# santimont/brpc-github-actions

Measured on AMD Instinct MI355X. Metric: echo QPS + p99 latency (rpc_press, 32B & 64KB body) at 1/2/4/8 MI355X, higher is better.
Workload: dtype uint8

## Files before the change

### brpc_amd/csrc/pb/descriptor.cc

```cpp
#include "pb/descriptor.h"

#include <string>

#include "pb/message.h"

namespace mrpc {
namespace pb {

Descriptor::~Descriptor() {
    if (owns_prototype) delete prototype;
}

const char* FieldTypeName(FieldType t) {
    switch (t) {
    case FieldType::DOUBLE: return "double";
    case FieldType::FLOAT: return "float";
    case FieldType::INT64: return "int64";
    case FieldType::UINT64: return "uint64";
    case FieldType::INT32: return "int32";
    case FieldType::FIXED64: return "fixed64";
    case FieldType::FIXED32: return "fixed32";
    case FieldType::BOOL: return "bool";
    case FieldType::STRING: return "string";
    case FieldType::GROUP: return "group";
// ... 28 lines not shown
size_t CppTypeAlign(CppType t) {
    switch (t) {
    case CppType::BOOL: return 1;
    case CppType::INT32:
    case CppType::UINT32:
    case CppType::ENUM:
    case CppType::FLOAT: return 4;
    default: return 8;
    }
}

std::string ToJsonName(const std::string& s) {
    std::string out;
    bool up = false;
    for (char c : s) {
        if (c == '_') {
            up = true;
        } else if (up) {
            out.push_back((char)toupper((unsigned char)c));
            up = false;
        } else {
            out.push_back(c);
        }
    }
    return out;
}

bool FieldDescriptor::is_map() const { return is_repeated() && message_type && message_type->map_entry; }

const EnumValueDescriptor* EnumDescriptor::FindValueByNumber(int n) const {
    for (auto& v : values) {
        if (v.number == n) return &v;
    }
    return nullptr;
}

const EnumValueDescriptor* EnumDescriptor::FindValueByName(const std::string& s) const {
    for (auto& v : values) {
        if (v.name == s) return &v;
    }
    return nullptr;
}

void Descriptor::BuildIndex() {
    _by_number.clear();
    _by_number_sparse.clear();
    _by_name.clear();
    for (size_t i = 0; i < fields.size(); ++i) {
        FieldDescriptor& f = fields[i];
        f.index = (int)i;
        f.containing_type = this;
        if (f.json_name.empty()) f.json_name = ToJsonName(f.name);
        if (f.number > 0 && f.number < 256) {
            if ((int)_by_number.size() <= f.number) _by_number.resize(f.number + 1, 0);
            _by_number[f.number] = (int)i + 1;
        } else {
            _by_number_sparse[f.number] = (int)i;
        }
        _by_name[f.name] = (int)i;
    }
}

const FieldDescriptor* Descriptor::FindFieldByNumber(int n) const {
    if (n > 0 && n < (int)_by_number.size()) {
        int i = _by_number[n];
        return i ? &fields[i - 1] : nullptr;
    }
    auto it = _by_number_sparse.find(n);
    return it == _by_number_sparse.end() ? nullptr : &fields[it->second];
}

const FieldDescriptor* Descriptor::FindFieldByName(const std::string& s) const {
    auto it = _by_name.find(s);
    return it == _by_name.end() ? nullptr : &fields[it->second];
}

const FieldDescriptor* Descriptor::FindFieldByJsonName(const std::string& s) const {
    for (auto& f : fields) {
        if (f.json_name == s) return &f;
    }
    return nullptr;
}

Message* Descriptor::NewMessage() const {
    if (factory) return factory();
    if (prototype) return prototype->New();
    return nullptr;
}

const MethodDescriptor* ServiceDescriptor::FindMethodByName(const std::string& n) const {
    for (auto& m : methods) {
        if (m.name == n) return &m;
    }
    return nullptr;
}

DescriptorPool* DescriptorPool::generated_pool() {
    static DescriptorPool* p = new DescriptorPool;
    return p;
}

void DescriptorPool::add_message(Descriptor* d) {
    _messages[d->full_name] = d;
    for (Descriptor* n : d->nested_types) add_message(n);
    for (EnumDescriptor* e : d->enum_types) _enums[e->full_name] = e;
}

void DescriptorPool::AddFile(FileDescriptor* f) {
    std::lock_guard<std::mutex> g(_mu);
    _files.emplace_back(f);
    _file_by_name[f->name] = f;
    for (Descriptor* d : f->message_types) add_message(d);
    for (EnumDescriptor* e : f->enum_types) _enums[e->full_name] = e;
    for (ServiceDescriptor* s : f->services) _services[s->full_name] = s;
}

const FileDescriptor* DescriptorPool::FindFileByName(const std::string& n) const {
    std::lock_guard<std::mutex> g(_mu);
    auto it = _file_by_name.find(n);
    return it == _file_by_name.end() ? nullptr : it->second;
}

static std::string strip_dot(const std::string& s) { return (!s.empty() && s[0] == '.') ? s.substr(1) : s; }

const Descriptor* DescriptorPool::FindMessageTypeByName(const std::string& n) const {
    std::lock_guard<std::mutex> g(_mu);
    auto it = _messages.find(strip_dot(n));
    return it == _messages.end() ? nullptr : it->second;
}

const EnumDescriptor* DescriptorPool::FindEnumTypeByName(const std::string& n) const {
    std::lock_guard<std::mutex> g(_mu);
    auto it = _enums.find(strip_dot(n));
    return it == _enums.end() ? nullptr : it->second;
}

const ServiceDescriptor* DescriptorPool::FindServiceByName(const std::string& n) const {
    std::lock_guard<std::mutex> g(_mu);
    auto it = _services.find(strip_dot(n));
    return it == _services.end() ? nullptr : it->second;
}

const MethodDescriptor* DescriptorPool::FindMethodByName(const std::string& n) const {
    std::string s = strip_dot(n);
    size_t dot = s.rfind('.');
    if (dot == std::string::npos) return nullptr;
    const ServiceDescriptor* sd = FindServiceByName(s.substr(0, dot));
    return sd ? sd->FindMethodByName(s.substr(dot + 1)) : nullptr;
}

std::vector<const FileDescriptor*> DescriptorPool::files() const {
    std::lock_guard<std::mutex> g(_mu);
    std::vector<const FileDescriptor*> out;
    for (auto& f : _files) out.push_back(f.get());
    return out;
}

std::vector<const ServiceDescriptor*> DescriptorPool::services() const {
    std::lock_guard<std::mutex> g(_mu);
    std::vector<const ServiceDescriptor*> out;
    for (auto& kv : _services) out.push_back(kv.second);
    return out;
}

}
}
// ... 1 lines not shown
```

### brpc_amd/csrc/pb/descriptor.h

```cpp
#pragma once

#include <atomic>

#include <cstdint>
#include <map>
#include <memory>
#include <mutex>
#include <string>
#include <vector>

namespace mrpc {
namespace pb {

class Message;
class Descriptor;
class EnumDescriptor;
class FileDescriptor;
class ServiceDescriptor;

enum class FieldType : uint8_t {
    DOUBLE = 1, FLOAT = 2, INT64 = 3, UINT64 = 4, INT32 = 5, FIXED64 = 6, FIXED32 = 7, BOOL = 8,
    STRING = 9, GROUP = 10, MESSAGE = 11, BYTES = 12, UINT32 = 13, ENUM = 14, SFIXED32 = 15,
    SFIXED64 = 16, SINT32 = 17, SINT64 = 18,
};
// ... 12 lines not shown
    return i < 19 ? kMap[i] : CppType::INT32;
}
size_t CppTypeSize(CppType t);
size_t CppTypeAlign(CppType t);

struct EnumValueDescriptor {
    std::string name;
    int number;
};

class EnumDescriptor {
public:
    std::string name;
    std::string full_name;
    const FileDescriptor* file = nullptr;
    std::vector<EnumValueDescriptor> values;
    const EnumValueDescriptor* FindValueByNumber(int n) const;
    const EnumValueDescriptor* FindValueByName(const std::string& s) const;
};

class FieldDescriptor {
public:
    std::string name;
    std::string json_name;
    int number = 0;
    FieldType type = FieldType::INT32;
    Label label = Label::OPTIONAL;
    bool packed = false;
    bool proto3_implicit = false;
    std::string type_name;
    const Descriptor* message_type = nullptr;
    const EnumDescriptor* enum_type = nullptr;
    const Descriptor* containing_type = nullptr;
    int index = 0;
    int oneof_index = -1;
    bool has_default = false;
    std::string default_str;
    int64_t default_int = 0;
    uint64_t default_uint = 0;
    double default_double = 0;
    std::string default_string;
    uint32_t offset = 0;
    int32_t has_bit = -1;
    std::map<std::string, std::string> options;

    bool is_repeated() const { return label == Label::REPEATED; }
    bool is_required() const { return label == Label::REQUIRED; }
    bool is_map() const;
    CppType cpp_type() const { return CppTypeOf(type); }
    bool is_packable() const { return cpp_type() != CppType::STRING && cpp_type() != CppType::MESSAGE; }
};

class Descriptor {
public:
    std::string name;
    std::string full_name;
    const FileDescriptor* file = nullptr;
    const Descriptor* containing_type = nullptr;
    std::vector<FieldDescriptor> fields;
    std::vector<std::string> oneof_names;
    std::vector<Descriptor*> nested_types;
    std::vector<EnumDescriptor*> enum_types;
    bool map_entry = false;
    bool proto3 = false;
    uint32_t has_bits_offset = 0;
    uint32_t num_has_bits = 0;
    uint32_t object_size = 0;
    Message* (*factory)() = nullptr;
    const Message* prototype = nullptr;
    bool owns_prototype = false;
    std::atomic<const void*> mcpack_handler{nullptr};
    Descriptor() = default;
    Descriptor(const Descriptor&) = delete;
    Descriptor& operator=(const Descriptor&) = delete;
    ~Descriptor();

    int field_count() const { return (int)fields.size(); }
    const FieldDescriptor* field(int i) const { return &fields[i]; }
    const FieldDescriptor* FindFieldByNumber(int n) const;
    const FieldDescriptor* FindFieldByName(const std::string& s) const;
    const FieldDescriptor* FindFieldByJsonName(const std::string& s) const;
    void BuildIndex();
    Message* NewMessage() const;

private:
    std::vector<int> _by_number;
    std::map<int, int> _by_number_sparse;
    std::map<std::string, int> _by_name;
};

class MethodDescriptor {
public:
    std::string name;
    std::string full_name;
    const ServiceDescriptor* service = nullptr;
    const Descriptor* input_type = nullptr;
    const Descriptor* output_type = nullptr;
    std::string input_type_name;
    std::string output_type_name;
    int index = 0;
    bool client_streaming = false;
    bool server_streaming = false;
    std::map<std::string, std::string> options;
};

class ServiceDescriptor {
public:
    std::string name;
    std::string full_name;
    const FileDescriptor* file = nullptr;
    std::vector<MethodDescriptor> methods;
    std::map<std::string, std::string> options;
    int method_count() const { return (int)methods.size(); }
    const MethodDescriptor* method(int i) const { return &methods[i]; }
    const MethodDescriptor* FindMethodByName(const std::string& n) const;
};

class FileDescriptor {
public:
    std::string name;
    std::string package;
    std::string syntax = "proto2";
    std::vector<std::string> dependencies;
    std::vector<Descriptor*> message_types;
    std::vector<EnumDescriptor*> enum_types;
    std::vector<ServiceDescriptor*> services;
    std::map<std::string, std::string> options;
    std::string source;
    std::vector<std::unique_ptr<Descriptor>> owned_messages;
    std::vector<std::unique_ptr<EnumDescriptor>> owned_enums;
    std::vector<std::unique_ptr<ServiceDescriptor>> owned_services;
};

class DescriptorPool {
public:
    static DescriptorPool* generated_pool();
    void AddFile(FileDescriptor* f);
    const FileDescriptor* FindFileByName(const std::string& n) const;
    const Descriptor* FindMessageTypeByName(const std::string& full_name) const;
    const EnumDescriptor* FindEnumTypeByName(const std::string& full_name) const;
    const ServiceDescriptor* FindServiceByName(const std::string& full_name) const;
    const MethodDescriptor* FindMethodByName(const std::string& full_name) const;
    std::vector<const FileDescriptor*> files() const;
    std::vector<const ServiceDescriptor*> services() const;

private:
    void add_message(Descriptor* d);
    mutable std::mutex _mu;
    std::vector<std::unique_ptr<FileDescriptor>> _files;
    std::map<std::string, const FileDescriptor*> _file_by_name;
    std::map<std::string, const Descriptor*> _messages;
    std::map<std::string, const EnumDescriptor*> _enums;
    std::map<std::string, const ServiceDescriptor*> _services;
};

std::string ToJsonName(const std::string& field_name);

}
}
```

### brpc_amd/csrc/pb/message.cc

```cpp
#include "pb/message.h"

#include <algorithm>
#include <cmath>
#include <cstdio>
#include <sstream>

#include "base/buf.h"
#include "base/logging.h"

namespace mrpc {
namespace pb {

namespace {

template <typename T>
inline T& ref(Message* m, const FieldDescriptor* f) {
    return *reinterpret_cast<T*>(reinterpret_cast<char*>(m) + f->offset);
}
template <typename T>
inline const T& cref(const Message& m, const FieldDescriptor* f) {
    return *reinterpret_cast<const T*>(reinterpret_cast<const char*>(&m) + f->offset);
}
inline uint32_t* has_bits(Message* m) {
    return reinterpret_cast<uint32_t*>(reinterpret_cast<char*>(m) + m->GetDescriptor()->has_bits_offset);
}
inline const uint32_t* has_bits(const Message& m) {
    return reinterpret_cast<const uint32_t*>(reinterpret_cast<const char*>(&m) + m.GetDescriptor()->has_bits_offset);
}

WireType wire_type_of(FieldType t) {
    switch (t) {
    case FieldType::DOUBLE:
    case FieldType::FIXED64:
    case FieldType::SFIXED64: return WIRETYPE_FIXED64;
    case FieldType::FLOAT:
    case FieldType::FIXED32:
    case FieldType::SFIXED32: return WIRETYPE_FIXED32;
    case FieldType::STRING:
    case FieldType::BYTES:
    case FieldType::MESSAGE: return WIRETYPE_LENGTH_DELIMITED;
    case FieldType::GROUP: return WIRETYPE_START_GROUP;
    default: return WIRETYPE_VARINT;
    }
}

size_t scalar_size(FieldType t, const void* p) {
    switch (t) {
    case FieldType::DOUBLE:
    case FieldType::FIXED64:
    case FieldType::SFIXED64: return 8;
    case FieldType::FLOAT:
    case FieldType::FIXED32:
    case FieldType::SFIXED32: return 4;
    case FieldType::BOOL: return 1;
    case FieldType::INT32:
    case FieldType::ENUM: return int32_size(*(const int32_t*)p);
    case FieldType::SINT32: return varint_size(zigzag32(*(const int32_t*)p));
    case FieldType::UINT32: return varint_size(*(const uint32_t*)p);
    case FieldType::INT64: return varint_size((uint64_t)*(const int64_t*)p);
    case FieldType::SINT64: return varint_size(zigzag64(*(const int64_t*)p));
    case FieldType::UINT64: return varint_size(*(const uint64_t*)p);
    default: return 0;
    }
}

uint8_t* write_scalar(uint8_t* o, FieldType t, const void* p) {
    switch (t) {
    case FieldType::DOUBLE:
    case FieldType::FIXED64:
    case FieldType::SFIXED64: return write_fixed64(o, *(const uint64_t*)p);
    case FieldType::FLOAT:
    case FieldType::FIXED32:
    case FieldType::SFIXED32: return write_fixed32(o, *(const uint32_t*)p);
    case FieldType::BOOL: *o++ = (*(const uint8_t*)p) ? 1 : 0; return o;
    case FieldType::INT32:
    case FieldType::ENUM: return write_varint(o, (uint64_t)(int64_t)*(const int32_t*)p);
    case FieldType::SINT32: return write_varint(o, zigzag32(*(const int32_t*)p));
    case FieldType::UINT32: return write_varint(o, *(const uint32_t*)p);
    case FieldType::INT64: return write_varint(o, (uint64_t)*(const int64_t*)p);
    case FieldType::SINT64: return write_varint(o, zigzag64(*(const int64_t*)p));
    case FieldType::UINT64: return write_varint(o, *(const uint64_t*)p);
    default: return o;
    }
}

inline size_t vsize64(uint64_t v) { return (size_t)(((63 - __builtin_clzll(v | 1)) * 9 + 73) >> 6); }
size_t repeated_payload_bytes(FieldType t, const char* data, size_t n) {
    size_t s = 0;
    switch (t) {
    case FieldType::DOUBLE:
    case FieldType::FIXED64:
    case FieldType::SFIXED64: return 8 * n;
    case FieldType::FLOAT:
    case FieldType::FIXED32:
    case FieldType::SFIXED32: return 4 * n;
    case FieldType::BOOL: return n;
    case FieldType::INT32:
    case FieldType::ENUM: {
        const int32_t* v = reinterpret_cast<const int32_t*>(data);
        for (size_t i = 0; i < n; ++i) s += vsize64((uint64_t)(int64_t)v[i]);
        return s;
    }
    case FieldType::SINT32: {
        const int32_t* v = reinterpret_cast<const int32_t*>(data);
        for (size_t i = 0; i < n; ++i) s += vsize64(zigzag32(v[i]));
        return s;
    }
    case FieldType::UINT32: {
        const uint32_t* v = reinterpret_cast<const uint32_t*>(data);
        for (size_t i = 0; i < n; ++i) s += vsize64(v[i]);
        return s;
    }
    case FieldType::INT64:
    case FieldType::UINT64: {
        const uint64_t* v = reinterpret_cast<const uint64_t*>(data);
        for (size_t i = 0; i < n; ++i) s += vsize64(v[i]);
        return s;
    }
    case FieldType::SINT64: {
        const int64_t* v = reinterpret_cast<const int64_t*>(data);
        for (size_t i = 0; i < n; ++i) s += vsize64(zigzag64(v[i]));
        return s;
    }
    default: return 0;
    }
}

size_t elem_bytes(FieldType t) {
    switch (CppTypeOf(t)) {
    case CppType::BOOL: return 1;
    case CppType::INT32:
    case CppType::UINT32:
    case CppType::ENUM:
    case CppType::FLOAT: return 4;
    default: return 8;
    }
}

struct RawVec {
    const char* data;
    size_t n;
};
RawVec raw_repeated(const Message& m, const FieldDescriptor* f) {
    const char* base = reinterpret_cast<const char*>(&m) + f->offset;
    switch (f->cpp_type()) {
    case CppType::BOOL: {
        auto& v = *(const std::vector<uint8_t>*)base;
        return RawVec{(const char*)v.data(), v.size()};
    }
    case CppType::INT32:
    case CppType::ENUM: {
        auto& v = *(const std::vector<int32_t>*)base;
        return RawVec{(const char*)v.data(), v.size()};
    }
    case CppType::UINT32: {
        auto& v = *(const std::vector<uint32_t>*)base;
        return RawVec{(const char*)v.data(), v.size()};
    }
    case CppType::FLOAT: {
        auto& v = *(const std::vector<float>*)base;
        return RawVec{(const char*)v.data(), v.size()};
    }
    case CppType::INT64: {
        auto& v = *(const std::vector<int64_t>*)base;
        return RawVec{(const char*)v.data(), v.size()};
    }
    case CppType::UINT64: {
        auto& v = *(const std::vector<uint64_t>*)base;
        return RawVec{(const char*)v.data(), v.size()};
    }
    case CppType::DOUBLE: {
        auto& v = *(const std::vector<double>*)base;
        return RawVec{(const char*)v.data(), v.size()};
    }
    default: return RawVec{nullptr, 0};
    }
}

bool is_default_scalar(const Message& m, const FieldDescriptor* f) {
    switch (f->cpp_type()) {
    case CppType::BOOL: return !cref<bool>(m, f);
    case CppType::INT32:
    case CppType::ENUM: return cref<int32_t>(m, f) == 0;
    case CppType::UINT32: return cref<uint32_t>(m, f) == 0;
    case CppType::FLOAT: {
        float v = cref<float>(m, f);
        uint32_t bits;
        memcpy(&bits, &v, 4);
        return bits == 0;
    }
    case CppType::INT64: return cref<int64_t>(m, f) == 0;
    case CppType::UINT64: return cref<uint64_t>(m, f) == 0;
    case CppType::DOUBLE: {
        double v = cref<double>(m, f);
        uint64_t bits;
        memcpy(&bits, &v, 8);
        return bits == 0;
    }
    case CppType::STRING: return cref<std::string>(m, f).empty();
    case CppType::MESSAGE: return cref<Message*>(m, f) == nullptr;
    }
    return true;
}

bool field_present(const Message& m, const FieldDescriptor* f) {
    if (f->cpp_type() == CppType::MESSAGE) return cref<Message*>(m, f) != nullptr;
    if (f->has_bit >= 0) return (has_bits(m)[f->has_bit >> 5] >> (f->has_bit & 31)) & 1;
    return !is_default_scalar(m, f);
}

// ... 41 lines not shown
    ref<std::vector<T>>(m, f).push_back(v);
}

void store_number(Message* m, const FieldDescriptor* f, uint64_t raw) {
    const bool rep = f->is_repeated();
    switch (f->type) {
    case FieldType::INT32:
    case FieldType::ENUM:
    case FieldType::SFIXED32: {
        int32_t v = (int32_t)raw;
        if (rep) push_raw<int32_t>(m, f, v); else ref<int32_t>(m, f) = v;
        break;
    }
    case FieldType::SINT32: {
        int32_t v = unzigzag32((uint32_t)raw);
        if (rep) push_raw<int32_t>(m, f, v); else ref<int32_t>(m, f) = v;
        break;
    }
    case FieldType::UINT32:
    case FieldType::FIXED32: {
        uint32_t v = (uint32_t)raw;
        if (rep) push_raw<uint32_t>(m, f, v); else ref<uint32_t>(m, f) = v;
        break;
    }
    case FieldType::INT64:
    case FieldType::SFIXED64: {
        int64_t v = (int64_t)raw;
        if (rep) push_raw<int64_t>(m, f, v); else ref<int64_t>(m, f) = v;
        break;
    }
    case FieldType::SINT64: {
        int64_t v = unzigzag64(raw);
        if (rep) push_raw<int64_t>(m, f, v); else ref<int64_t>(m, f) = v;
        break;
    }
    case FieldType::UINT64:
    case FieldType::FIXED64: {
        if (rep) push_raw<uint64_t>(m, f, raw); else ref<uint64_t>(m, f) = raw;
        break;
    }
    case FieldType::BOOL: {
        uint8_t v = raw != 0;
        if (rep) push_raw<uint8_t>(m, f, v); else ref<bool>(m, f) = v;
        break;
    }
    case FieldType::FLOAT: {
        uint32_t b = (uint32_t)raw;
        float v;
        memcpy(&v, &b, 4);
        if (rep) push_raw<float>(m, f, v); else ref<float>(m, f) = v;
        break;
    }
    case FieldType::DOUBLE: {
        double v;
        memcpy(&v, &raw, 8);
        if (rep) push_raw<double>(m, f, v); else ref<double>(m, f) = v;
        break;
    }
    default: break;
    }
    if (!rep) {
        if (f->oneof_index >= 0) ClearOneofSiblings(m, f);
        set_has(m, f);
    }
}

bool read_number(CodedInput* in, FieldType t, uint64_t* out) {
    switch (wire_type_of(t)) {
    case WIRETYPE_VARINT: return in->read_varint(out);
    case WIRETYPE_FIXED32: {
        uint32_t v;
        if (!in->read_fixed32(&v)) return false;
        *out = v;
        return true;
    }
    case WIRETYPE_FIXED64: return in->read_fixed64(out);
    default: return false;
    }
}

bool parse_message(Message* m, CodedInput* in);

template <typename T, typename Conv>
bool bulk_varints(Message* m, const FieldDescriptor* f, const uint8_t* p, size_t len, Conv conv) {
    size_t n = 0;
    for (size_t i = 0; i < len; ++i) n += (p[i] >> 7) ^ 1;
    auto& vec = ref<std::vector<T>>(m, f);
    const size_t base = vec.size();
    vec.resize(base + n);
    T* out = vec.data() + base;
    CodedInput in(p, len);
    for (size_t k = 0; k < n; ++k) {
        uint64_t v;
        if (!in.read_varint(&v)) {
            vec.resize(base + k);
            return false;
        }
        out[k] = conv(v);
    }
    return in.at_limit();
}

template <typename T>
bool bulk_fixed(Message* m, const FieldDescriptor* f, const uint8_t* p, size_t len) {
    if (len % sizeof(T)) return false;
    auto& vec = ref<std::vector<T>>(m, f);
    const size_t base = vec.size();
    vec.resize(base + len / sizeof(T));
    memcpy(vec.data() + base, p, len);
    return true;
}

bool parse_packed(Message* m, const FieldDescriptor* f, const uint8_t* p, size_t len) {
    switch (f->type) {
    case FieldType::INT32:
    case FieldType::ENUM: return bulk_varints<int32_t>(m, f, p, len, [](uint64_t v) { return (int32_t)v; });
    case FieldType::SINT32:
        return bulk_varints<int32_t>(m, f, p, len, [](uint64_t v) { return unzigzag32((uint32_t)v); });
    case FieldType::UINT32: return bulk_varints<uint32_t>(m, f, p, len, [](uint64_t v) { return (uint32_t)v; });
    case FieldType::INT64: return bulk_varints<int64_t>(m, f, p, len, [](uint64_t v) { return (int64_t)v; });
    case FieldType::SINT64: return bulk_varints<int64_t>(m, f, p, len, [](uint64_t v) { return unzigzag64(v); });
    case FieldType::UINT64: return bulk_varints<uint64_t>(m, f, p, len, [](uint64_t v) { return v; });
    case FieldType::BOOL: return bulk_varints<uint8_t>(m, f, p, len, [](uint64_t v) { return (uint8_t)(v != 0); });
    case FieldType::FIXED32:
    case FieldType::SFIXED32: return f->cpp_type() == CppType::UINT32 ? bulk_fixed<uint32_t>(m, f, p, len)
                                                                      : bulk_fixed<int32_t>(m, f, p, len);
    case FieldType::FIXED64: return bulk_fixed<uint64_t>(m, f, p, len);
    case FieldType::SFIXED64: return bulk_fixed<int64_t>(m, f, p, len);
    case FieldType::FLOAT: return bulk_fixed<float>(m, f, p, len);
    case FieldType::DOUBLE: return bulk_fixed<double>(m, f, p, len);
    default: return false;
    }
}

bool parse_field(Message* m, const FieldDescriptor* f, uint32_t tag, CodedInput* in) {
    const WireType wt = (WireType)(tag & 7);
    const WireType expected = wire_type_of(f->type);
    if (f->is_repeated() && f->is_packable() && wt == WIRETYPE_LENGTH_DELIMITED) {
        uint64_t len;
        const uint8_t* p;
        if (!in->read_varint(&len) || !in->read_bytes((size_t)len, &p)) return false;
        return parse_packed(m, f, p, (size_t)len);
    }
    if (wt != expected) {
        return in->skip_field(tag, m->mutable_unknown_fields());
    }
    switch (f->cpp_type()) {
    case CppType::STRING: {
        uint64_t len;
        const uint8_t* d;
        if (!in->read_varint(&len) || !in->read_bytes((size_t)len, &d)) return false;
        if (f->is_repeated()) {
            ref<std::vector<std::string>>(m, f).emplace_back((const char*)d, (size_t)len);
        } else {
            if (f->oneof_index >= 0) ClearOneofSiblings(m, f);
            ref<std::string>(m, f).assign((const char*)d, (size_t)len);
            set_has(m, f);
        }
        return true;
    }
    case CppType::MESSAGE: {
        if (f->type == FieldType::GROUP) return in->skip_field(tag, m->mutable_unknown_fields());
        uint64_t len;
        const uint8_t* old;
        if (!in->read_varint(&len) || !in->push_limit((size_t)len, &old)) return false;
        Message* sub = f->is_repeated() ? Reflection::AddMessage(m, f) : Reflection::MutableMessage(m, f);
        if (!in->inc_depth()) return false;
        if (!parse_message(sub, in)) return false;
        in->dec_depth();
        if (!in->at_limit()) return false;
        in->pop_limit(old);
        return true;
    }
    default: {
        uint64_t v;
        if (!read_number(in, f->type, &v)) return false;
        store_number(m, f, v);
        return true;
    }
    }
}

bool parse_message(Message* m, CodedInput* in) { return m->MergePartialFromCodedInput(in); }

}


Message::~Message() {}

void Message::Clear() {
    const Descriptor* d = GetDescriptor();
    for (const FieldDescriptor& fd : d->fields) {
        const FieldDescriptor* f = &fd;
        if (f->is_repeated()) {
            clear_repeated(this, f);
        } else if (f->cpp_type() == CppType::MESSAGE) {
            Message*& sub = ref<Message*>(this, f);
            if (sub) sub->Clear();
            delete sub;
            sub = nullptr;
        } else {
            set_scalar_default(this, f);
        }
    }
    uint32_t* hb = has_bits(this);
    for (uint32_t i = 0; i < (d->num_has_bits + 31) / 32; ++i) hb[i] = 0;
    _unknown.clear();
}

size_t Message::ByteSizeLong() const {
    const Descriptor* d = GetDescriptor();
    size_t total = 0;
    for (const FieldDescriptor& fd : d->fields) {
        const FieldDescriptor* f = &fd;
        const size_t tag_size = varint_size(make_tag(f->number, WIRETYPE_VARINT));
        if (f->is_repeated()) {
            switch (f->cpp_type()) {
            case CppType::STRING: {
                const auto& v = cref<std::vector<std::string>>(*this, f);
                for (const auto& s : v) total += tag_size + varint_size(s.size()) + s.size();
                break;
            }
            case CppType::MESSAGE: {
                const auto& v = cref<RepeatedPtrBase>(*this, f);
                for (int i = 0; i < v.size(); ++i) {
                    size_t s = v.Get(i)->ByteSizeLong();
                    total += tag_size + varint_size(s) + s;
                }
                break;
            }
            default: {
                RawVec rv = raw_repeated(*this, f);
                if (rv.n == 0) break;
                const size_t data = repeated_payload_bytes(f->type, rv.data, rv.n);
                if (f->packed) total += tag_size + varint_size(data) + data;
                else total += tag_size * rv.n + data;
            }
            }
            continue;
        }
        if (!field_present(*this, f)) continue;
        switch (f->cpp_type()) {
        case CppType::STRING: {
            const auto& s = cref<std::string>(*this, f);
            total += tag_size + varint_size(s.size()) + s.size();
            break;
        }
        case CppType::MESSAGE: {
            size_t s = cref<Message*>(*this, f)->ByteSizeLong();
            total += tag_size + varint_size(s) + s;
            break;
        }
        default:
            total += tag_size + scalar_size(f->type, reinterpret_cast<const char*>(this) + f->offset);
        }
    }
    total += _unknown.size();
    _cached_size = (int)total;
    return total;
}

const void* Reflection::RepeatedScalarData(const Message& m, const FieldDescriptor* f, size_t* n, size_t* eb) {
    *n = 0;
    *eb = 0;
    if (!f->is_repeated() || f->cpp_type() == CppType::STRING || f->cpp_type() == CppType::MESSAGE) return nullptr;
    RawVec rv = raw_repeated(m, f);
    *n = rv.n;
    *eb = elem_bytes(f->type);
    return rv.data;
}

static thread_local PackedRunSink* tls_run_sink = nullptr;

PackedRunSink* SetThreadPackedRunSink(PackedRunSink* sink) {
    PackedRunSink* prev = tls_run_sink;
    tls_run_sink = sink;
    return prev;
}

bool IsVarintFieldType(FieldType t) {
    switch (t) {
    case FieldType::INT32:
    case FieldType::ENUM:
    case FieldType::SINT32:
    case FieldType::UINT32:
    case FieldType::INT64:
    case FieldType::SINT64:
    case FieldType::UINT64:
    case FieldType::BOOL: return true;
    default: return false;
    }
}

void EncodePackedRunOnHost(const PackedRun& run) {
    uint8_t* o = run.dst;
    const char* v = static_cast<const char*>(run.values);
    for (size_t i = 0; i < run.n; ++i) o = write_scalar(o, run.type, v + i * run.elem_bytes);
}

uint8_t* Message::SerializeWithCachedSizesToArray(uint8_t* o) const {
    const Descriptor* d = GetDescriptor();
    for (const FieldDescriptor& fd : d->fields) {
        const FieldDescriptor* f = &fd;
        if (f->is_repeated()) {
            switch (f->cpp_type()) {
            case CppType::STRING: {
                for (const auto& s : cref<std::vector<std::string>>(*this, f)) {
                    o = write_tag(o, f->number, WIRETYPE_LENGTH_DELIMITED);
                    o = write_varint(o, s.size());
                    memcpy(o, s.data(), s.size());
                    o += s.size();
                }
                break;
            }
            case CppType::MESSAGE: {
                const auto& v = cref<RepeatedPtrBase>(*this, f);
                for (int i = 0; i < v.size(); ++i) {
                    const Message* sub = v.Get(i);
                    o = write_tag(o, f->number, WIRETYPE_LENGTH_DELIMITED);
                    o = write_varint(o, (uint64_t)sub->GetCachedSize());
                    o = sub->SerializeWithCachedSizesToArray(o);
                }
                break;
            }
            default: {
                RawVec rv = raw_repeated(*this, f);
                if (rv.n == 0) break;
                const size_t eb = elem_bytes(f->type);
                PackedRunSink* sink = tls_run_sink;
                if (f->packed && sink && rv.n >= sink->min_elems() && IsVarintFieldType(f->type)) {
                    PackedRun run;
                    run.values = rv.data;
                    run.n = rv.n;
                    run.elem_bytes = eb;
                    run.type = f->type;
                    run.chunk_bytes.reserve((rv.n + kPackedRunChunkElems - 1) / kPackedRunChunkElems);
                    size_t data = 0;
                    for (size_t c = 0; c < rv.n; c += kPackedRunChunkElems) {
                        const size_t e = std::min(rv.n, c + kPackedRunChunkElems);
                        const size_t cb = repeated_payload_bytes(f->type, rv.data + c * eb, e - c);
                        run.chunk_bytes.push_back((uint32_t)cb);
                        data += cb;
                    }
                    o = write_tag(o, f->number, WIRETYPE_LENGTH_DELIMITED);
                    o = write_varint(o, data);
                    run.dst = o;
                    run.bytes = data;
                    o += data;
                    sink->Take(std::move(run));
                } else if (f->packed) {
                    const size_t data = repeated_payload_bytes(f->type, rv.data, rv.n);
                    o = write_tag(o, f->number, WIRETYPE_LENGTH_DELIMITED);
                    o = write_varint(o, data);
                    for (size_t i = 0; i < rv.n; ++i) o = write_scalar(o, f->type, rv.data + i * eb);
                } else {
                    const WireType wt = wire_type_of(f->type);
                    for (size_t i = 0; i < rv.n; ++i) {
                        o = write_tag(o, f->number, wt);
                        o = write_scalar(o, f->type, rv.data + i * eb);
                    }
                }
            }
            }
            continue;
        }
        if (!field_present(*this, f)) continue;
        switch (f->cpp_type()) {
        case CppType::STRING: {
            const auto& s = cref<std::string>(*this, f);
            o = write_tag(o, f->number, WIRETYPE_LENGTH_DELIMITED);
            o = write_varint(o, s.size());
            memcpy(o, s.data(), s.size());
            o += s.size();
            break;
        }
        case CppType::MESSAGE: {
            const Message* sub = cref<Message*>(*this, f);
            o = write_tag(o, f->number, WIRETYPE_LENGTH_DELIMITED);
            o = write_varint(o, (uint64_t)sub->GetCachedSize());
            o = sub->SerializeWithCachedSizesToArray(o);
            break;
        }
        default:
            o = write_tag(o, f->number, wire_type_of(f->type));
            o = write_scalar(o, f->type, reinterpret_cast<const char*>(this) + f->offset);
        }
    }
    if (!_unknown.empty()) {
        memcpy(o, _unknown.data(), _unknown.size());
        o += _unknown.size();
    }
    return o;
}

bool Message::MergePartialFromCodedInput(CodedInput* in) {
    const Descriptor* d = GetDescriptor();
    for (;;) {
        const uint32_t tag = in->read_tag();
        if (tag == 0) return true;
        if (tag == 0xFFFFFFFFu || (tag >> 3) == 0) return false;
        if ((tag & 7) == WIRETYPE_END_GROUP) return false;
        const FieldDescriptor* f = d->FindFieldByNumber((int)(tag >> 3));
        if (!f) {
            if (!in->skip_field(tag, &_unknown)) return false;
            continue;
        }
        if (!parse_field(this, f, tag, in)) return false;
    }
}

static bool is_initialized_impl(const Message& m, std::string* missing, const std::string& prefix) {
    bool ok = true;
    const Descriptor* d = m.GetDescriptor();
    for (const FieldDescriptor& fd : d->fields) {
        const FieldDescriptor* f = &fd;
        if (f->is_required() && !field_present(m, f)) {
            ok = false;
            if (missing) {
                if (!missing->empty()) missing->append(", ");
                missing->append(prefix + f->name);
            } else {
                return false;
            }
        }
        if (f->cpp_type() == CppType::MESSAGE) {
            if (f->is_repeated()) {
                const auto& v = cref<RepeatedPtrBase>(m, f);
                for (int i = 0; i < v.size(); ++i) {
                    if (!is_initialized_impl(*v.Get(i), missing, prefix + f->name + "[" + std::to_string(i) + "].")) {
                        ok = false;
                        if (!missing) return false;
                    }
                }
            } else if (const Message* sub = cref<Message*>(m, f)) {
                if (!is_initialized_impl(*sub, missing, prefix + f->name + ".")) {
                    ok = false;
                    if (!missing) return false;
                }
            }
        }
    }
    return ok;
}

bool Message::IsInitialized() const { return is_initialized_impl(*this, nullptr, ""); }

std::string Message::InitializationErrorString() const {
    std::string s;
    is_initialized_impl(*this, &s, "");
    return s;
}

void Message::MergeFrom(const Message& from) {
    const Descriptor* d = GetDescriptor();
    CHECK(d == from.GetDescriptor() || d->full_name == from.GetDescriptor()->full_name)
        << "MergeFrom between different types";
    for (const FieldDescriptor& fd : d->fields) {
        const FieldDescriptor* f = &fd;
        if (f->is_repeated()) {
            const int n = Reflection::FieldSize(from, f);
            for (int i = 0; i < n; ++i) {
                switch (f->cpp_type()) {
                case CppType::INT32: Reflection::AddInt32(this, f, Reflection::GetRepeatedInt32(from, f, i)); break;
                case CppType::ENUM: Reflection::AddEnumValue(this, f, Reflection::GetRepeatedEnumValue(from, f, i)); break;
                case CppType::UINT32: Reflection::AddUInt32(this, f, Reflection::GetRepeatedUInt32(from, f, i)); break;
                case CppType::INT64: Reflection::AddInt64(this, f, Reflection::GetRepeatedInt64(from, f, i)); break;
                case CppType::UINT64: Reflection::AddUInt64(this, f, Reflection::GetRepeatedUInt64(from, f, i)); break;
                case CppType::FLOAT: Reflection::AddFloat(this, f, Reflection::GetRepeatedFloat(from, f, i)); break;
                case CppType::DOUBLE: Reflection::AddDouble(this, f, Reflection::GetRepeatedDouble(from, f, i)); break;
                case CppType::BOOL: Reflection::AddBool(this, f, Reflection::GetRepeatedBool(from, f, i)); break;
                case CppType::STRING: Reflection::AddString(this, f, Reflection::GetRepeatedString(from, f, i)); break;
                case CppType::MESSAGE: Reflection::AddMessage(this, f)->MergeFrom(Reflection::GetRepeatedMessage(from, f, i)); break;
                }
            }
            continue;
        }
        if (!field_present(from, f)) continue;
        switch (f->cpp_type()) {
        case CppType::MESSAGE: Reflection::MutableMessage(this, f)->MergeFrom(*cref<Message*>(from, f)); break;
        case CppType::STRING: Reflection::SetString(this, f, cref<std::string>(from, f)); break;
        default:
            memcpy(reinterpret_cast<char*>(this) + f->offset, reinterpret_cast<const char*>(&from) + f->offset,
                   CppTypeSize(f->cpp_type()));
            if (f->oneof_index >= 0) ClearOneofSiblings(this, f);
            set_has(this, f);
        }
    }
    _unknown.append(from._unknown);
}

void Message::CopyFrom(const Message& from) {
    if (&from == this) return;
    Clear();
    MergeFrom(from);
}

bool Message::SerializeToArray(void* data, int size) const {
    const size_t n = ByteSizeLong();
    if ((size_t)size < n) return false;
    SerializeWithCachedSizesToArray((uint8_t*)data);
    return true;
}

bool Message::AppendToString(std::string* out) const {
    const size_t n = ByteSizeLong();
    const size_t old = out->size();
    out->resize(old + n);
    uint8_t* e = SerializeWithCachedSizesToArray((uint8_t*)&(*out)[old]);
    return (size_t)(e - (uint8_t*)&(*out)[old]) == n;
}

bool Message::SerializeToString(std::string* out) const {
    out->clear();
    return AppendToString(out);
}

std::string Message::SerializeAsString() const {
    std::string s;
    SerializeToString(&s);
    return s;
}

bool Message::SerializeToBuf(Buf* out) const {
    const size_t n = ByteSizeLong();
    if (n == 0) return true;
    char* p = out->append_contiguous(n);
    if (!p) return false;
    uint8_t* e = SerializeWithCachedSizesToArray((uint8_t*)p);
// ... 323 lines not shown
```

### brpc_amd/csrc/pb/message.h

```cpp
#pragma once

#include <cstdint>
#include <string>
#include <vector>

#include "pb/descriptor.h"
#include "pb/wire.h"

namespace mrpc {
class Buf;
namespace pb {

class Message {
public:
    Message() : _cached_size(0) {}
    virtual ~Message();
    virtual const Descriptor* GetDescriptor() const = 0;
    virtual Message* New() const = 0;

    virtual void Clear();
    virtual size_t ByteSizeLong() const;
    virtual uint8_t* SerializeWithCachedSizesToArray(uint8_t* target) const;
    virtual bool MergePartialFromCodedInput(CodedInput* in);

    int ByteSize() const { return (int)ByteSizeLong(); }
    int GetCachedSize() const { return _cached_size; }
    void SetCachedSize(int s) const { _cached_size = s; }

    bool IsInitialized() const;
    std::string InitializationErrorString() const;
    void CopyFrom(const Message& from);
    void MergeFrom(const Message& from);

    bool SerializeToString(std::string* out) const;
    std::string SerializeAsString() const;
    bool SerializeToArray(void* data, int size) const;
    bool AppendToString(std::string* out) const;
    bool SerializeToBuf(Buf* out) const;
    bool ParseFromArray(const void* data, size_t size);
    bool ParsePartialFromArray(const void* data, size_t size);
    bool ParseFromString(const std::string& s) { return ParseFromArray(s.data(), s.size()); }
    bool MergeFromString(const std::string& s);
    bool ParseFromBuf(const Buf& in);
    bool MergeFromFieldTable(const uint8_t* data, size_t size, const uint64_t* fields, int nfields,
                             class PackedRunDecoder* decoder = nullptr);
    std::string DebugString() const;
    std::string ShortDebugString() const;
    std::string GetTypeName() const { return GetDescriptor()->full_name; }

    const std::string& unknown_fields() const { return _unknown; }
    std::string* mutable_unknown_fields() { return &_unknown; }

protected:
    mutable int _cached_size;
    std::string _unknown;
};

class RepeatedPtrBase {
public:
    RepeatedPtrBase() {}
    ~RepeatedPtrBase() { Clear(); }
    RepeatedPtrBase(const RepeatedPtrBase&) = delete;
    RepeatedPtrBase& operator=(const RepeatedPtrBase&) = delete;
    int size() const { return (int)_v.size(); }
    bool empty() const { return _v.empty(); }
    void Clear() {
        for (Message* m : _v) delete m;
        _v.clear();
    }
    Message* AddMessage(const Message* prototype) {
        Message* m = prototype->New();
        _v.push_back(m);
        return m;
    }
    void AddAllocated(Message* m) { _v.push_back(m); }
    Message* Get(int i) const { return _v[i]; }
    void RemoveLast() {
        delete _v.back();
        _v.pop_back();
    }
    void SwapElements(int a, int b) { std::swap(_v[a], _v[b]); }
    std::vector<Message*>& raw() { return _v; }
    const std::vector<Message*>& raw() const { return _v; }

protected:
    std::vector<Message*> _v;
};

template <typename T>
class RepeatedPtrField : public RepeatedPtrBase {
public:
    T* Add() {
        T* t = new T;
        _v.push_back(t);
        return t;
    }
    const T& Get(int i) const { return *static_cast<const T*>(_v[i]); }
    T* Mutable(int i) { return static_cast<T*>(_v[i]); }
    const T& operator[](int i) const { return Get(i); }
    class const_iterator {
    public:
        explicit const_iterator(std::vector<Message*>::const_iterator it) : _it(it) {}
        const T& operator*() const { return *static_cast<const T*>(*_it); }
        const T* operator->() const { return static_cast<const T*>(*_it); }
        const_iterator& operator++() { ++_it; return *this; }
        bool operator!=(const const_iterator& o) const { return _it != o._it; }
    private:
        std::vector<Message*>::const_iterator _it;
    };
    const_iterator begin() const { return const_iterator(_v.begin()); }
    const_iterator end() const { return const_iterator(_v.end()); }
};
// ... 98 lines not shown
```

### build.py

```python
#!/usr/bin/env python3
import argparse
import glob
import os
import shutil
import subprocess
import sys
import sysconfig

ROOT = os.path.dirname(os.path.abspath(__file__))
PKG = os.path.join(ROOT, "brpc_amd")
CSRC = os.path.join(PKG, "csrc")
BUILD = os.path.join(ROOT, "build")
GEN = os.path.join(BUILD, "gen")
ROCM = os.environ.get("ROCM_PATH", "/opt/rocm")
ARCH = os.environ.get("PYTORCH_ROCM_ARCH", "gfx950").split(";")[0]

BOOT_DIRS = ["base", "pb"]
MCPACK_PROTOS = ["echo", "test_services"]
NON_LIB_DIRS = {"tools", "python", "tests", "examples", "heapprof"}


def rel(p):
    return os.path.relpath(p, BUILD)

# ... 73 lines not shown
      "  depfile = $out.d\n  deps = gcc\n  description = CXX $in\n")
    w("rule hip\n  command = $hipcc $hipflags -MMD -MF $out.d -c $in -o $out\n"
      "  depfile = $out.d\n  deps = gcc\n  description = HIP $in\n")
    w("rule ar\n  command = rm -f $out && ar rcs $out $in\n  description = AR $out\n")
    w(f"rule solink\n  command = $cxx -shared {san} -o $out $in $extra $ldlibs\n  description = SO $out\n")
    w(f"rule link\n  command = $cxx {san} -o $out $in $extra $ldlibs\n  description = LINK $out\n")
    w("rule protoc\n  command = $protoc --cpp_out=$gendir --proto_path=$protodir $in\n"
      "  description = PROTOC $in\n")

    def cxx(src, extra="", implicit=()):
        o = obj_of(src)
        imp = (" | " + " ".join(x if x == "gen_headers" else rel(x) for x in implicit)) if implicit else ""
        w(f"build {rel(o)}: cxx {rel(src)}{imp}\n" + (f"  extra = {extra}\n" if extra else ""))
        return o

    boot_objs = [cxx(s) for s in boot_srcs]
    boot_lib = os.path.join(BUILD, "libmrpc_boot.a")
    w(f"build {rel(boot_lib)}: ar {' '.join(rel(o) for o in boot_objs)}\n")
    protoc = os.path.join(BUILD, "bin", "mrpc_protoc")
    protoc_main = cxx(os.path.join(CSRC, "tools", "protoc_main.cc"))
    w(f"build {rel(protoc)}: link {rel(protoc_main)} {rel(boot_lib)}\n")
    for p, cc, h in zip(protos, gen_ccs, gen_hs):
        w(f"build {rel(cc)} {rel(h)}: protoc {rel(p)} | {rel(protoc)}\n"
          f"  protoc = {rel(protoc)}\n  gendir = {rel(os.path.join(GEN, 'mrpc', 'proto'))}\n"
          f"  protodir = {rel(os.path.join(PKG, 'proto'))}\n")
    w("rule protoc_mcpack\n  command = $protoc --mcpack_out=$gendir --proto_path=$protodir $in\n"
      "  description = PROTOC-MCPACK $in\n")
    for p in protos:
        b = os.path.splitext(os.path.basename(p))[0]
        if b not in MCPACK_PROTOS:
            continue
        mc = os.path.join(GEN, "mrpc", "proto", b + ".pb.mcpack.cc")
        w(f"build {rel(mc)}: protoc_mcpack {rel(p)} | {rel(protoc)}\n"
          f"  protoc = {rel(protoc)}\n  gendir = {rel(os.path.join(GEN, 'mrpc', 'proto'))}\n"
          f"  protodir = {rel(os.path.join(PKG, 'proto'))}\n")
        gen_ccs.append(mc)
    w(f"build gen_headers: phony {' '.join(rel(h) for h in gen_hs)}\n")

    lib_objs = []
    for s in lib_srcs:
        if os.path.relpath(s, CSRC).split(os.sep)[0] in BOOT_DIRS:
            lib_objs.append(obj_of(s))
        else:
            lib_objs.append(cxx(s, implicit=["gen_headers"]))
    for cc in gen_ccs:
        lib_objs.append(cxx(cc, implicit=["gen_headers"]))
    for s in hip_srcs:
        o = obj_of(s)
        w(f"build {rel(o)}: hip {rel(s)} | gen_headers\n")
        lib_objs.append(o)
    libso = os.path.join(PKG, "lib", "libmrpc.so")
    w(f"build {rel(libso)}: solink {' '.join(rel(o) for o in lib_objs)}\n")

    rpath = "-Wl,-rpath,'$$ORIGIN/../../brpc_amd/lib' -Wl,-rpath,'$$ORIGIN/lib'"
    linkmrpc = f"-L{rel(os.path.join(PKG, 'lib'))} -lmrpc {rpath}"

    py_srcs = sorted(glob.glob(os.path.join(CSRC, "python", "*.cc")))
    py_objs = [cxx(s, extra=f"-isystem {pybind_inc} -isystem {pyinc} -fvisibility=hidden",
                   implicit=["gen_headers"]) for s in py_srcs]
    pymod = os.path.join(PKG, "_native" + ext_suffix)
    w(f"build {rel(pymod)}: solink {' '.join(rel(o) for o in py_objs)} | {rel(libso)}\n"
      f"  extra = {linkmrpc}\n")

    ut_srcs = sorted(glob.glob(os.path.join(CSRC, "tests", "*.cc")))
    ut_objs = [cxx(s, implicit=["gen_headers"]) for s in ut_srcs]
    bins = []
    if ut_objs:
        ut = os.path.join(BUILD, "bin", "mrpc_unittests")
        w(f"build {rel(ut)}: link {' '.join(rel(o) for o in ut_objs)} | {rel(libso)}\n  extra = {linkmrpc}\n")
        bins.append(ut)
    for s in sorted(glob.glob(os.path.join(CSRC, "tests", "stub", "*.cc"))):
        name = os.path.splitext(os.path.basename(s))[0]
        o = cxx(s, extra="-fvisibility=hidden")
        so = os.path.join(BUILD, "lib", "lib%s.so" % name)
        w(f"build {rel(so)}: solink {rel(o)}\n  ldlibs = -lpthread\n")
        bins.append(so)
    for s in sorted(glob.glob(os.path.join(CSRC, "tools", "*.cc"))):
        name = os.path.splitext(os.path.basename(s))[0]
        if name == "protoc_main":
            continue
        o = cxx(s, implicit=["gen_headers"])
        b = os.path.join(BUILD, "bin", name)
        w(f"build {rel(b)}: link {rel(o)} | {rel(libso)}\n  extra = {linkmrpc}\n")
        bins.append(b)
    for d in sorted(glob.glob(os.path.join(CSRC, "examples", "*"))):
        if not os.path.isdir(d):
            continue
        for s in sorted(glob.glob(os.path.join(d, "*.cc"))):
            name = os.path.basename(d) + "_" + os.path.splitext(os.path.basename(s))[0]
            o = cxx(s, implicit=["gen_headers"])
            b = os.path.join(BUILD, "bin", name)
            w(f"build {rel(b)}: link {rel(o)} | {rel(libso)}\n  extra = {linkmrpc}\n")
            bins.append(b)
    hp = os.path.join(CSRC, "heapprof", "heapprof.cc")
    if os.path.exists(hp):
        hp_o = cxx(hp)
        hp_so = os.path.join(PKG, "lib", "libmrpc_heapprof.so")
        w(f"build {rel(hp_so)}: solink {rel(hp_o)}\n  ldlibs = -ldl -lpthread\n")
        d_o = cxx(os.path.join(CSRC, "heapprof", "heapprof_demo.cc"), implicit=["gen_headers"])
        b = os.path.join(BUILD, "bin", "heapprof_demo")
        w(f"build {rel(b)}: link {rel(d_o)} {rel(hp_o)} | {rel(libso)}\n  extra = {linkmrpc} -rdynamic\n")
        bins += [hp_so, b]
    w(f"build all: phony {rel(libso)} {rel(pymod)} {' '.join(rel(b) for b in bins)}\n")
    w("default all\n")
    with open(os.path.join(BUILD, "build.ninja"), "w") as f:
        f.write("\n".join(L))
    cmd = ["ninja", "-C", BUILD, f"-j{a.j}"] + a.targets
    r = subprocess.run(cmd)
    sys.exit(r.returncode)


if __name__ == "__main__":
    main()
```

Before: 1.704 million.

## Add generated-codec support helpers and cache required-field check per descriptor

```diff
diff --git a/brpc_amd/csrc/pb/descriptor.cc b/brpc_amd/csrc/pb/descriptor.cc
--- a/brpc_amd/csrc/pb/descriptor.cc
+++ b/brpc_amd/csrc/pb/descriptor.cc
@@ -134,6 +134,30 @@
     return nullptr;
 }
 
+static bool reaches_required(const Descriptor* d, std::vector<const Descriptor*>* seen) {
+    for (const Descriptor* s : *seen) {
+        if (s == d) return false;
+    }
+    seen->push_back(d);
+    for (const FieldDescriptor& f : d->fields) {
+        if (f.is_required()) return true;
+    }
+    for (const FieldDescriptor& f : d->fields) {
+        if (f.message_type && reaches_required(f.message_type, seen)) return true;
+    }
+    return false;
+}
+
+bool Descriptor::HasRequiredFields() const {
+    int v = _has_required.load(std::memory_order_relaxed);
+    if (v < 0) {
+        std::vector<const Descriptor*> seen;
+        v = reaches_required(this, &seen) ? 1 : 0;
+        _has_required.store(v, std::memory_order_relaxed);
+    }
+    return v != 0;
+}
+
 Message* Descriptor::NewMessage() const {
     if (factory) return factory();
     if (prototype) return prototype->New();
diff --git a/brpc_amd/csrc/pb/descriptor.h b/brpc_amd/csrc/pb/descriptor.h
--- a/brpc_amd/csrc/pb/descriptor.h
+++ b/brpc_amd/csrc/pb/descriptor.h
@@ -118,11 +118,13 @@
     const FieldDescriptor* FindFieldByJsonName(const std::string& s) const;
     void BuildIndex();
     Message* NewMessage() const;
+    bool HasRequiredFields() const;
 
 private:
     std::vector<int> _by_number;
     std::map<int, int> _by_number_sparse;
     std::map<std::string, int> _by_name;
+    mutable std::atomic<int> _has_required{-1};
 };
 
 class MethodDescriptor {
diff --git a/brpc_amd/csrc/pb/generated_support.h b/brpc_amd/csrc/pb/generated_support.h
--- /dev/null
+++ b/brpc_amd/csrc/pb/generated_support.h
@@ -0,0 +1,63 @@
+#pragma once
+
+#include <cstdint>
+#include <cstring>
+
+#include "base/flags.h"
+#include "pb/message.h"
+#include "pb/wire.h"
+
+DECLARE_bool(pb_generated_codecs);
+
+namespace mrpc {
+namespace pb {
+namespace gen {
+
+inline bool enabled() { return __builtin_expect(FLAGS_pb_generated_codecs, 1); }
+
+bool ParseFieldSlow(Message* m, const Descriptor* d, uint32_t tag, CodedInput* in);
+
+bool AppendPacked(FieldType t, void* vec, const uint8_t* p, size_t len);
+
+size_t RepeatedPayloadBytes(FieldType t, const void* data, size_t n);
+
+uint8_t* WritePackedField(uint8_t* o, int number, FieldType t, const void* data, size_t n);
+
+inline uint8_t* WriteFloat(uint8_t* o, float v) {
+    memcpy(o, &v, 4);
+    return o + 4;
+}
+inline uint8_t* WriteDouble(uint8_t* o, double v) {
+    memcpy(o, &v, 8);
+    return o + 8;
+}
+inline float FloatFromBits(uint32_t b) {
+    float v;
+    memcpy(&v, &b, 4);
+    return v;
+}
+inline double DoubleFromBits(uint64_t b) {
+    double v;
+    memcpy(&v, &b, 8);
+    return v;
+}
+inline bool NonZeroBits(float v) {
+    uint32_t b;
+    memcpy(&b, &v, 4);
+    return b != 0;
+}
+inline bool NonZeroBits(double v) {
+    uint64_t b;
+    memcpy(&b, &v, 8);
+    return b != 0;
+}
+inline uint8_t* WriteBytes(uint8_t* o, const std::string& s) {
+    o = write_varint(o, s.size());
+    memcpy(o, s.data(), s.size());
+    return o + s.size();
+}
+inline size_t BytesSize(const std::string& s) { return varint_size(s.size()) + s.size(); }
+
+}
+}
+}
diff --git a/brpc_amd/csrc/pb/message.cc b/brpc_amd/csrc/pb/message.cc
--- a/brpc_amd/csrc/pb/message.cc
+++ b/brpc_amd/csrc/pb/message.cc
@@ -7,6 +7,12 @@
 
 #include "base/buf.h"
 #include "base/logging.h"
+#include "pb/generated_support.h"
+
+DEFINE_bool(pb_generated_codecs, true,
+            "Messages generated by mrpc_protoc run their generated codec; false: the "
+            "descriptor-driven one (same bytes, the control of an A/B)");
+MRPC_VALIDATE_FLAG(pb_generated_codecs, mrpc::PassValidator);
 
 namespace mrpc {
 namespace pb {
@@ -126,6 +132,34 @@
     }
 }
 
+template <typename T, typename Conv>
+inline uint8_t* write_varints(uint8_t* o, const char* data, size_t n, Conv conv) {
+    const T* v = reinterpret_cast<const T*>(data);
+    for (size_t i = 0; i < n; ++i) o = write_varint(o, conv(v[i]));
+    return o;
+}
+uint8_t* write_repeated_payload(uint8_t* o, FieldType t, const char* data, size_t n) {
+    switch (t) {
+    case FieldType::DOUBLE:
+    case FieldType::FIXED64:
+    case FieldType::SFIXED64: memcpy(o, data, 8 * n); return o + 8 * n;
+    case FieldType::FLOAT:
+    case FieldType::FIXED32:
+    case FieldType::SFIXED32: memcpy(o, data, 4 * n); return o + 4 * n;
+    case FieldType::BOOL:
+        for (size_t i = 0; i < n; ++i) *o++ = data[i] ? 1 : 0;
+        return o;
+    case FieldType::INT32:
+    case FieldType::ENUM: return write_varints<int32_t>(o, data, n, [](int32_t v) { return (uint64_t)(int64_t)v; });
+    case FieldType::SINT32: return write_varints<int32_t>(o, data, n, [](int32_t v) { return (uint64_t)zigzag32(v); });
+    case FieldType::UINT32: return write_varints<uint32_t>(o, data, n, [](uint32_t v) { return (uint64_t)v; });
+    case FieldType::INT64:
+    case FieldType::UINT64: return write_varints<uint64_t>(o, data, n, [](uint64_t v) { return v; });
+    case FieldType::SINT64: return write_varints<int64_t>(o, data, n, [](int64_t v) { return zigzag64(v); });
+    default: return o;
+    }
+}
+
 size_t elem_bytes(FieldType t) {
     switch (CppTypeOf(t)) {
     case CppType::BOOL: return 1;
@@ -333,55 +367,69 @@
 bool parse_message(Message* m, CodedInput* in);
 
 template <typename T, typename Conv>
-bool bulk_varints(Message* m, const FieldDescriptor* f, const uint8_t* p, size_t len, Conv conv) {
+bool bulk_varints(void* vecp, const uint8_t* p, size_t len, Conv conv) {
     size_t n = 0;
     for (size_t i = 0; i < len; ++i) n += (p[i] >> 7) ^ 1;
-    auto& vec = ref<std::vector<T>>(m, f);
+    auto& vec = *static_cast<std::vector<T>*>(vecp);
     const size_t base = vec.size();
     vec.resize(base + n);
     T* out = vec.data() + base;
-    CodedInput in(p, len);
+    const uint8_t* q = p;
+    const uint8_t* const end = p + len;
     for (size_t k = 0; k < n; ++k) {
-        uint64_t v;
-        if (!in.read_varint(&v)) {
-            vec.resize(base + k);
-            return false;
+        uint64_t v = *q++;
+        if (v >= 0x80) {
+            v &= 0x7f;
+            int shift = 7;
+            for (;;) {
+                if (shift >= 70 || q >= end) {
+                    vec.resize(base + k);
+                    return false;
+                }
+                const uint8_t b = *q++;
+                v |= (uint64_t)(b & 0x7f) << (shift & 63);
+                if (!(b & 0x80)) break;
+                shift += 7;
+            }
         }
         out[k] = conv(v);
     }
-    return in.at_limit();
+    return q == end;
 }
 
 template <typename T>
-bool bulk_fixed(Message* m, const FieldDescriptor* f, const uint8_t* p, size_t len) {
+bool bulk_fixed(void* vecp, const uint8_t* p, size_t len) {
     if (len % sizeof(T)) return false;
-    auto& vec = ref<std::vector<T>>(m, f);
+    auto& vec = *static_cast<std::vector<T>*>(vecp);
     const size_t base = vec.size();
     vec.resize(base + len / sizeof(T));
     memcpy(vec.data() + base, p, len);
     return true;
 }
 
+bool parse_packed_into(FieldType t, void* vec, const uint8_t* p, size_t len) {
+    switch (t) {
+    case FieldType::INT32:
+    case FieldType::ENUM: return bulk_varints<int32_t>(vec, p, len, [](uint64_t v) { return (int32_t)v; });
+    case FieldType::SINT32:
+        return bulk_varints<int32_t>(vec, p, len, [](uint64_t v) { return unzigzag32((uint32_t)v); });
+    case FieldType::UINT32: return bulk_varints<uint32_t>(vec, p, len, [](uint64_t v) { return (uint32_t)v; });
+    case FieldType::INT64: return bulk_varints<int64_t>(vec, p, len, [](uint64_t v) { return (int64_t)v; });
+    case FieldType::SINT64: return bulk_varints<int64_t>(vec, p, len, [](uint64_t v) { return unzigzag64(v); });
+    case FieldType::UINT64: return bulk_varints<uint64_t>(vec, p, len, [](uint64_t v) { return v; });
+    case FieldType::BOOL: return bulk_varints<uint8_t>(vec, p, len, [](uint64_t v) { return (uint8_t)(v != 0); });
+    case FieldType::FIXED32: return bulk_fixed<uint32_t>(vec, p, len);
+    case FieldType::SFIXED32: return bulk_fixed<int32_t>(vec, p, len);
+    case FieldType::FIXED64: return bulk_fixed<uint64_t>(vec, p, len);
+    case FieldType::SFIXED64: return bulk_fixed<int64_t>(vec, p, len);
+    case FieldType::FLOAT: return bulk_fixed<float>(vec, p, len);
+    case FieldType::DOUBLE: return bulk_fixed<double>(vec, p, len);
+    default: return false;
+    }
+}
+
 bool parse_packed(Message* m, const FieldDescriptor* f, const uint8_t* p, size_t len) {
-    switch (f->type) {
-    case FieldType::INT32:
-    case FieldType::ENUM: return bulk_varints<int32_t>(m, f, p, len, [](uint64_t v) { return (int32_t)v; });
-    case FieldType::SINT32:
-        return bulk_varints<int32_t>(m, f, p, len, [](uint64_t v) { return unzigzag32((uint32_t)v); });
-    case FieldType::UINT32: return bulk_varints<uint32_t>(m, f, p, len, [](uint64_t v) { return (uint32_t)v; });
-    case FieldType::INT64: return bulk_varints<int64_t>(m, f, p, len, [](uint64_t v) { return (int64_t)v; });
-    case FieldType::SINT64: return bulk_varints<int64_t>(m, f, p, len, [](uint64_t v) { return unzigzag64(v); });
-    case FieldType::UINT64: return bulk_varints<uint64_t>(m, f, p, len, [](uint64_t v) { return v; });
-    case FieldType::BOOL: return bulk_varints<uint8_t>(m, f, p, len, [](uint64_t v) { return (uint8_t)(v != 0); });
-    case FieldType::FIXED32:
-    case FieldType::SFIXED32: return f->cpp_type() == CppType::UINT32 ? bulk_fixed<uint32_t>(m, f, p, len)
-                                                                      : bulk_fixed<int32_t>(m, f, p, len);
-    case FieldType::FIXED64: return bulk_fixed<uint64_t>(m, f, p, len);
-    case FieldType::SFIXED64: return bulk_fixed<int64_t>(m, f, p, len);
-    case FieldType::FLOAT: return bulk_fixed<float>(m, f, p, len);
-    case FieldType::DOUBLE: return bulk_fixed<double>(m, f, p, len);
-    default: return false;
-    }
+    return parse_packed_into(f->type, reinterpret_cast<char*>(m) + f->offset, p, len);
 }
 
 bool parse_field(Message* m, const FieldDescriptor* f, uint32_t tag, CodedInput* in) {
@@ -544,9 +592,57 @@
 }
 
 void EncodePackedRunOnHost(const PackedRun& run) {
-    uint8_t* o = run.dst;
-    const char* v = static_cast<const char*>(run.values);
-    for (size_t i = 0; i < run.n; ++i) o = write_scalar(o, run.type, v + i * run.elem_bytes);
+    if (run.n) write_repeated_payload(run.dst, run.type, static_cast<const char*>(run.values), run.n);
+}
+
+namespace gen {
+
+uint8_t* WritePackedField(uint8_t* o, int number, FieldType t, const void* values, size_t n) {
+    const char* data = static_cast<const char*>(values);
+    const size_t eb = elem_bytes(t);
+    PackedRunSink* sink = tls_run_sink;
+    if (sink && n >= sink->min_elems() && IsVarintFieldType(t)) {
+        PackedRun run;
+        run.values = data;
+        run.n = n;
+        run.elem_bytes = eb;
+        run.type = t;
+        run.chunk_bytes.reserve((n + kPackedRunChunkElems - 1) / kPackedRunChunkElems);
+        size_t bytes = 0;
+        for (size_t c = 0; c < n; c += kPackedRunChunkElems) {
+            const size_t e = std::min(n, c + kPackedRunChunkElems);
+            const size_t cb = repeated_payload_bytes(t, data + c * eb, e - c);
+            run.chunk_bytes.push_back((uint32_t)cb);
+            bytes += cb;
+        }
+        o = write_tag(o, number, WIRETYPE_LENGTH_DELIMITED);
+        o = write_varint(o, bytes);
+        run.dst = o;
+        run.bytes = bytes;
+        o += bytes;
+        sink->Take(std::move(run));
+        return o;
+    }
+    const size_t bytes = repeated_payload_bytes(t, data, n);
+    o = write_tag(o, number, WIRETYPE_LENGTH_DELIMITED);
+    o = write_varint(o, bytes);
+    return write_repeated_payload(o, t, data, n);
+}
+
+size_t RepeatedPayloadBytes(FieldType t, const void* data, size_t n) {
+    return repeated_payload_bytes(t, static_cast<const char*>(data), n);
+}
+
+bool AppendPacked(FieldType t, void* vec, const uint8_t* p, size_t len) { return parse_packed_into(t, vec, p, len); }
+
+bool ParseFieldSlow(Message* m, const Descriptor* d, uint32_t tag, CodedInput* in) {
+    if (tag == 0xFFFFFFFFu || (tag >> 3) == 0) return false;
+    if ((tag & 7) == WIRETYPE_END_GROUP) return false;
+    const FieldDescriptor* f = d->FindFieldByNumber((int)(tag >> 3));
+    if (!f) return in->skip_field(tag, m->mutable_unknown_fields());
+    return parse_field(m, f, tag, in);
+}
+
 }
 
 uint8_t* Message::SerializeWithCachedSizesToArray(uint8_t* o) const {
@@ -577,34 +673,10 @@
             default: {
                 RawVec rv = raw_repeated(*this, f);
                 if (rv.n == 0) break;
-                const size_t eb = elem_bytes(f->type);
-                PackedRunSink* sink = tls_run_sink;
-                if (f->packed && sink && rv.n >= sink->min_elems() && IsVarintFieldType(f->type)) {
-                    PackedRun run;
-                    run.values = rv.data;
-                    run.n = rv.n;
-                    run.elem_bytes = eb;
-                    run.type = f->type;
-                    run.chunk_bytes.reserve((rv.n + kPackedRunChunkElems - 1) / kPackedRunChunkElems);
-                    size_t data = 0;
-                    for (size_t c = 0; c < rv.n; c += kPackedRunChunkElems) {
-                        const size_t e = std::min(rv.n, c + kPackedRunChunkElems);
-                        const size_t cb = repeated_payload_bytes(f->type, rv.data + c * eb, e - c);
-                        run.chunk_bytes.push_back((uint32_t)cb);
-                        data += cb;
-                    }
-                    o = write_tag(o, f->number, WIRETYPE_LENGTH_DELIMITED);
-                    o = write_varint(o, data);
-                    run.dst = o;
-                    run.bytes = data;
-                    o += data;
-                    sink->Take(std::move(run));
-                } else if (f->packed) {
-                    const size_t data = repeated_payload_bytes(f->type, rv.data, rv.n);
-                    o = write_tag(o, f->number, WIRETYPE_LENGTH_DELIMITED);
-                    o = write_varint(o, data);
-                    for (size_t i = 0; i < rv.n; ++i) o = write_scalar(o, f->type, rv.data + i * eb);
+                if (f->packed) {
+                    o = gen::WritePackedField(o, f->number, f->type, rv.data, rv.n);
                 } else {
+                    const size_t eb = elem_bytes(f->type);
                     const WireType wt = wire_type_of(f->type);
                     for (size_t i = 0; i < rv.n; ++i) {
                         o = write_tag(o, f->number, wt);
@@ -694,7 +766,10 @@
     return ok;
 }
 
-bool Message::IsInitialized() const { return is_initialized_impl(*this, nullptr, ""); }
+bool Message::CheckInitialized() const {
+    if (!GetDescriptor()->HasRequiredFields()) return true;
+    return is_initialized_impl(*this, nullptr, "");
+}
 
 std::string Message::InitializationErrorString() const {
     std::string s;
diff --git a/brpc_amd/csrc/pb/message.h b/brpc_amd/csrc/pb/message.h
--- a/brpc_amd/csrc/pb/message.h
+++ b/brpc_amd/csrc/pb/message.h
@@ -27,7 +27,8 @@
     int GetCachedSize() const { return _cached_size; }
     void SetCachedSize(int s) const { _cached_size = s; }
 
-    bool IsInitialized() const;
+    bool IsInitialized() const { return CheckInitialized(); }
+    virtual bool CheckInitialized() const;
     std::string InitializationErrorString() const;
     void CopyFrom(const Message& from);
     void MergeFrom(const Message& from);
diff --git a/build.py b/build.py
--- a/build.py
+++ b/build.py
@@ -179,6 +179,15 @@
         o = cxx(s, implicit=["gen_headers"])
         b = os.path.join(BUILD, "bin", name)
         w(f"build {rel(b)}: link {rel(o)} | {rel(libso)}\n  extra = {linkmrpc}\n")
+        bins.append(b)
+    cb = os.path.join(ROOT, "benchmarks", "pb_codec_bench.cc")
+    if os.path.exists(cb):
+        cb_gen = [obj_of(os.path.join(GEN, "mrpc", "proto", n + ".pb.cc"))
+                  for n in ("echo", "rpc_meta", "options", "streaming_rpc_meta", "device_payload")]
+        o = cxx(cb, implicit=["gen_headers"])
+        b = os.path.join(BUILD, "bin", "pb_codec_bench")
+        w(f"build {rel(b)}: link {rel(o)} {' '.join(rel(x) for x in cb_gen)} {rel(boot_lib)}\n"
+          f"  ldlibs = -lpthread\n")
         bins.append(b)
     for d in sorted(glob.glob(os.path.join(CSRC, "examples", "*"))):
         if not os.path.isdir(d):
```

After: 1.764 million, median of 5. 1.03x the previous value.
